# kvas7andy/unreal

Hardware: NVIDIA B200
Metric: maze env-steps/s incl. pixel-change+returns (higher is better)
Workload: dtype f32

## Files before the change

include/unreal_b200.h:

```cpp
#ifndef UNREAL_B200_H_
#define UNREAL_B200_H_

#include <stdint.h>

#ifdef __cplusplus
extern "C" {
#endif

#define UNREAL_OK 0
#define UNREAL_EINVAL (-1)
#define UNREAL_ECUDA (-2)
#define UNREAL_ESTATE (-3)
#define UNREAL_ENOMEM (-4)

#define UNREAL_F32 0
#define UNREAL_U8 1
#define UNREAL_BF16 2

#define UNREAL_MAZE_GRID 7
#define UNREAL_FRAME_HW 84
#define UNREAL_PC_CELLS 20
#define UNREAL_MT_WORDS 624

const char* unreal_last_error(void);
int unreal_abi_version(void);
int unreal_device_info(int* sm_count, int* cc_major, int* cc_minor);
int unreal_set_tunable(const char* name, int value);
int unreal_get_tunable(const char* name, int* value);

int unreal_maze_set_map(const char* map49_host);
int unreal_maze_get_layout(int* start_x, int* start_y, int* goal_x, int* goal_y, uint8_t* walls49_host);

int unreal_maze_reset(int32_t* pos , int32_t* last_action , float* last_reward ,
                      const uint8_t* mask , int n, void* stream);

int unreal_maze_step(int32_t* pos, const int32_t* action , const uint8_t* active,
                     float* reward , uint8_t* terminal , int32_t* last_action,
                     float* last_reward, void* obs, int obs_dtype, float* pc, uint64_t* frame_rec,
                     int n, int auto_reset, void* stream);

int unreal_maze_window(int32_t* pos, const int32_t* action, float* reward, uint8_t* terminal, int32_t* last_action,
                       float* last_reward, void* obs, int obs_dtype, float* pc, uint64_t* frame_rec, int n, int t,
                       int auto_reset, void* stream);

int unreal_maze_render(const int32_t* pos, void* obs, int obs_dtype, int m, void* stream);

int unreal_maze_pixel_change(const int32_t* pos0, const int32_t* pos1, float* pc, int m, void* stream);
int unreal_maze_pc_targets(const int32_t* pos0, const int32_t* pos1, const int32_t* len, const float* boot, float gamma_pc,
                           float* tgt, int t, int n, void* stream);

int unreal_pixel_change(const void* cur, const void* prev, int dtype, float* pc, int m, int h, int w,
                        int c, void* stream);
int unreal_selfcheck_arith(unsigned long long* mismatches, void* stream);
int unreal_subsample(const float* a, float* out, int m, int h, int w, int width, void* stream);
int unreal_pixel_change_stream(const void* frames, int dtype, float* pc, int s, int l, int h, int w,
                               int c, void* stream);

int unreal_nstep_returns(const float* r, const float* v, const uint8_t* term, const float* boot,
                         float gamma, float* out_R, float* out_adv, int t, int n, void* stream);
int unreal_sequence_returns(const float* r, const int32_t* len, const float* boot, float gamma,
                            float* out_R , int n, int l, void* stream);

int unreal_pc_targets(const float* pc, const uint8_t* term, const int32_t* len, const float* boot,
                      float gamma_pc, float* tgt, int t, int n, void* stream);

int unreal_mt_seed(uint32_t* mt, int32_t* mt_pos, const uint32_t* seeds , int n, void* stream);
int unreal_choose_action(uint32_t* mt, int32_t* mt_pos, const float* pi, const uint8_t* active,
                         int32_t* action, int n, int a, void* stream);
int unreal_mt_randint(uint32_t* mt, int32_t* mt_pos, uint32_t high, int32_t* out, int n, int k, void* stream);

typedef struct unreal_replay unreal_replay_t;
int unreal_replay_create(unreal_replay_t** out, int n_envs, int history_size);
int unreal_replay_destroy(unreal_replay_t* r);
int unreal_replay_reset(unreal_replay_t* r, void* stream);
int unreal_replay_add(unreal_replay_t* r, const uint64_t* frame_rec , void* stream);
int unreal_replay_state(unreal_replay_t* r, uint8_t* full, int32_t* count, int64_t* top,
                        int32_t* n_pos, int32_t* n_neg, void* stream);
int unreal_replay_copy(unreal_replay_t* r, int direction, uint64_t* rec, int64_t* top, int32_t* count,
                       int32_t* n_pos, int32_t* n_neg, void* stream);
int unreal_replay_sample_sequence(unreal_replay_t* r, uint32_t* mt, int32_t* mt_pos, int seq_len,
                                  int32_t* start, int32_t* len, uint64_t* rec, void* stream);
int unreal_replay_sample_rp(unreal_replay_t* r, uint32_t* mt, int32_t* mt_pos, int32_t* start,
                            uint64_t* rec, void* stream);
int unreal_frame_unpack(const uint64_t* rec, int m, int32_t* pos0, int32_t* pos1, int32_t* action,
                        float* reward, uint8_t* terminal, int32_t* last_action, float* last_reward,
                        uint8_t* valid, void* stream);

int unreal_frame_pack(const int32_t* action, const float* reward, const uint8_t* terminal,
                      const int32_t* last_action , const float* last_reward ,
                      const uint8_t* active , uint64_t* rec, int n, void* stream);
int unreal_replay_add_slots(unreal_replay_t* r, const uint64_t* frame_rec, int32_t* slot, void* stream);
int unreal_ring_store(void* payload, const void* src, const int32_t* slot, int n_envs, int history_size,
                      long long item_bytes, void* stream);
int unreal_rows_select(void* out, const void* src, const int64_t* idx, const uint8_t* mask, int n, long long item_bytes,
                       void* stream);
int unreal_replay_gather(unreal_replay_t* r, const void* payload, long long item_bytes, const int32_t* start,
                         const int32_t* len , int seq_len, int time_major, void* out, void* stream);

int unreal_rollout_lar(const int32_t* last_action, const float* last_reward, const float* objective, int n, int a, int g,
                       float* lar, void* stream);
int unreal_rollout_post(const float* reward, const uint8_t* terminal, const uint64_t* frame_rec, int n, uint8_t* active,
                        uint8_t* ended, uint64_t* last_rec, float* episode_reward, float* lstm_c, float* lstm_h,
// ... 124 lines not shown
```

unreal_b200/_lib.py:

```python
import ctypes
import os
from ctypes import POINTER, c_char_p, c_double, c_float, c_int, c_int32, c_int64, c_uint8, c_uint32, c_void_p

import torch

HERE = os.path.dirname(os.path.abspath(__file__))
LIB_PATH = os.path.join(HERE, "libunreal_b200.so")

OK = 0
F32 = 0
U8 = 1


class UnrealError(RuntimeError):
  pass


if not os.path.exists(LIB_PATH):
  raise ImportError(
      "%s is missing: build it with `python -m unreal_b200.build` (nvcc, sm_100a). "
      "unreal_b200 has no CPU fallback." % LIB_PATH)

lib = ctypes.CDLL(LIB_PATH)

P = c_void_p

SIGNATURES = {
    "unreal_last_error": (c_char_p, []),
    "unreal_abi_version": (c_int, []),
    "unreal_device_info": (c_int, [POINTER(c_int), POINTER(c_int), POINTER(c_int)]),
    "unreal_set_tunable": (c_int, [c_char_p, c_int]),
    "unreal_get_tunable": (c_int, [c_char_p, POINTER(c_int)]),
    "unreal_maze_set_map": (c_int, [c_char_p]),
    "unreal_maze_get_layout": (c_int, [POINTER(c_int)] * 4 + [POINTER(c_uint8)]),
    "unreal_maze_reset": (c_int, [P, P, P, P, c_int, P]),
    "unreal_maze_step": (c_int, [P, P, P, P, P, P, P, P, c_int, P, P, c_int, c_int, P]),
    "unreal_maze_window": (c_int, [P, P, P, P, P, P, P, c_int, P, P, c_int, c_int, c_int, P]),
    "unreal_maze_render": (c_int, [P, P, c_int, c_int, P]),
    "unreal_maze_pixel_change": (c_int, [P, P, P, c_int, P]),
    "unreal_maze_pc_targets": (c_int, [P, P, P, P, c_float, P, c_int, c_int, P]),
    "unreal_pixel_change": (c_int, [P, P, c_int, P, c_int, c_int, c_int, c_int, P]),
    "unreal_pixel_change_stream": (c_int, [P, c_int, P, c_int, c_int, c_int, c_int, c_int, P]),
    "unreal_selfcheck_arith": (c_int, [P, P]),
    "unreal_subsample": (c_int, [P, P, c_int, c_int, c_int, c_int, P]),
    "unreal_nstep_returns": (c_int, [P, P, P, P, c_float, P, P, c_int, c_int, P]),
    "unreal_sequence_returns": (c_int, [P, P, P, c_float, P, c_int, c_int, P]),
    "unreal_pc_targets": (c_int, [P, P, P, P, c_float, P, c_int, c_int, P]),
    "unreal_mt_seed": (c_int, [P, P, P, c_int, P]),
    "unreal_choose_action": (c_int, [P, P, P, P, P, c_int, c_int, P]),
    "unreal_mt_randint": (c_int, [P, P, c_uint32, P, c_int, c_int, P]),
    "unreal_replay_create": (c_int, [POINTER(c_void_p), c_int, c_int]),
    "unreal_replay_destroy": (c_int, [c_void_p]),
    "unreal_replay_reset": (c_int, [c_void_p, P]),
    "unreal_replay_add": (c_int, [c_void_p, P, P]),
    "unreal_replay_state": (c_int, [c_void_p, P, P, P, P, P, P]),
    "unreal_replay_copy": (c_int, [c_void_p, c_int, P, P, P, P, P, P]),
    "unreal_replay_sample_sequence": (c_int, [c_void_p, P, P, c_int, P, P, P, P]),
    "unreal_replay_sample_rp": (c_int, [c_void_p, P, P, P, P, P]),
    "unreal_frame_unpack": (c_int, [P, c_int, P, P, P, P, P, P, P, P, P]),
    "unreal_frame_pack": (c_int, [P, P, P, P, P, P, P, c_int, P]),
    "unreal_replay_add_slots": (c_int, [c_void_p, P, P, P]),
    "unreal_ring_store": (c_int, [P, P, P, c_int, c_int, c_int64, P]),
    "unreal_rows_select": (c_int, [P, P, P, P, c_int, c_int64, P]),
    "unreal_replay_gather": (c_int, [c_void_p, P, c_int64, P, P, c_int, c_int, P, P]),
    "unreal_rollout_lar": (c_int, [P, P, P, c_int, c_int, c_int, P, P]),
    "unreal_rollout_post": (c_int, [P, P, P, c_int, P, P, P, P, P, P, P, P]),
    "unreal_maze_eval_act": (c_int, [P, c_int, c_int, P, P, P, P, P, P, P, P, P, P, P, P, c_int, c_int, P, P, P, P, c_int64,
                                     c_int, c_int, P]),
    "unreal_grad_sumsq": (c_int, [P, c_int64, P, P]),
    "unreal_rmsprop_update": (c_int, [P, P, P, P, c_int64, P, c_float, c_float, c_float, c_float, c_float,
                                      c_float, P, P]),
    "unreal_rmsprop_update_dlr": (c_int, [P, P, P, P, c_int64, P, c_float, P, c_float, c_float, c_float,
                                          c_float, P, P]),
    "unreal_gemm_bf16": (c_int, [P, c_int64, c_int, P, c_int64, c_int, P, c_int64, c_int, P, P, c_int, c_int, c_int,
                                 c_int, c_int, c_int, P]),
    "unreal_im2col": (c_int, [P, c_int, P, c_int, c_int, c_int, c_int, c_int, c_int, c_int, P]),
    "unreal_col2im": (c_int, [P, c_int, P, c_int, P, c_int, c_int, c_int, c_int, c_int, c_int, c_int, c_int, P]),
    "unreal_lstm_cell_fwd": (c_int, [P, P, P, P, P, c_int, P]),
    "unreal_lstm_cell_fwd_ld": (c_int, [P, P, P, P, P, c_int, c_int, P]),
    "unreal_lstm_cell_act": (c_int, [P, P, P, P, P, c_int, P]),
    "unreal_lstm_cell_fwd_g16": (c_int, [P, P, P, P, P, c_int, c_int, P]),
    "unreal_lstm_cell_act_g16": (c_int, [P, P, P, P, P, c_int, P]),
    "unreal_lstm_cell_act_heads": (c_int, [P, P, P, P, c_int, P, P, P, P, c_int, P, P, P]),
    "unreal_lstm_cell_bwd_g16": (c_int, [P, P, P, P, P, P, P, c_int, P]),
    "unreal_lstm_step_fwd": (c_int, [P, c_int64, P, P, P, P, P, P, P, c_int, P, P, c_int, c_int, c_int, P]),
    "unreal_lstm_step_bwd": (c_int, [P, P, c_int64, P, P, P, P, P, P, P, c_int, c_int, P]),
    "unreal_lstm_cell_bwd": (c_int, [P, P, P, P, P, P, c_int, P]),
    "unreal_lstm_cell_bwd2": (c_int, [P, P, P, P, P, P, P, c_int, P]),
    "unreal_s2d_frames": (c_int, [P, c_int, P, c_int, P]),
    "unreal_conv_fwd": (c_int, [P, c_int, P, P, P, c_int, P]),
    "unreal_relu_grad": (c_int, [P, c_int, P, P, P, c_int64, c_int, c_int, P]),
    "unreal_conv1_wgrad": (c_int, [P, P, P, c_int, P]),
    "unreal_conv2_wgrad": (c_int, [P, P, P, c_int, P]),
# ... 118 lines not shown
```

unreal_b200/csrc/maze.cu:

```cuda
#include "common.cuh"
#include "maze_core.cuh"

namespace unreal {

__constant__ MazeLayout c_maze;
static MazeLayout h_maze;
static bool h_maze_ready = false;

static const char kReferenceMap[] =
    "--+---G"
    "--+-+++"
    "S-+---+"
    "--+++--"
    "--+-+--"
    "--+----"
    "-----++";

constexpr int kFrameElems = UNREAL_FRAME_HW * UNREAL_FRAME_HW * 3;
constexpr int kRowElems = UNREAL_FRAME_HW * 3;
constexpr int kPcElems = UNREAL_PC_CELLS * UNREAL_PC_CELLS;
constexpr int kThreads = 256;

struct StepArgs {
  int32_t* pos;
// ... 1 lines not shown
  const uint8_t* active;
  float* reward;
  uint8_t* terminal;
  int32_t* last_action;
  float* last_reward;
  void* obs;
  float* pc;
  uint64_t* rec;
  int n;
  int auto_reset;
};

struct EnvInfo {
  int rx, ry;
  int x0, y0, x1, y1;
  int live;
};

template <bool kStep>
__device__ __forceinline__ EnvInfo env_logic(const StepArgs& a, int e) {
  EnvInfo o;
  int x = a.pos[2 * e], y = a.pos[2 * e + 1];
  o.rx = x; o.ry = y; o.x0 = x; o.y0 = y; o.x1 = x; o.y1 = y; o.live = 1;
  if (!kStep) return o;
  if (a.active != nullptr && a.active[e] == 0) {
    o.live = 0;
    a.reward[e] = 0.f;
    a.terminal[e] = 0;
    if (a.rec) a.rec[e] = 0ull;
    return o;
  }
  int act = a.action[e];
  MazeStep s = maze_step_core(c_maze, x, y, act);
  int la = a.last_action[e];
  float lr = a.last_reward[e];
  if (a.rec) a.rec[e] = frame_pack(x, y, s.x1, s.y1, act, s.reward, s.terminal, la, (int)lr);
  a.reward[e] = (float)s.reward;
  a.terminal[e] = (uint8_t)s.terminal;
  o.x1 = s.x1; o.y1 = s.y1;
  if (s.terminal && a.auto_reset) {
    o.rx = c_maze.start_x; o.ry = c_maze.start_y;
    a.last_action[e] = 0;
    a.last_reward[e] = 0.f;
  } else {
    o.rx = s.x1; o.ry = s.y1;
    a.last_action[e] = act;
    a.last_reward[e] = (float)s.reward;
  }
  a.pos[2 * e] = o.rx;
  a.pos[2 * e + 1] = o.ry;
  return o;
}

__device__ __forceinline__ float4 pc_value4(int x0, int y0, int x1, int y1, int q) {
  int i = q / 5, j0 = (q - i * 5) * 4;
  bool moved = (x0 != x1) || (y0 != y1);
  int wy0 = pc_overlap(i, y0), wy1 = pc_overlap(i, y1);
  if (!moved || (wy0 | wy1) == 0) return make_float4(0.f, 0.f, 0.f, 0.f);
  float v[4];
#pragma unroll
  for (int u = 0; u < 4; ++u) {
    const float k = (float)(wy0 * pc_overlap(j0 + u, x0) + wy1 * pc_overlap(j0 + u, x1));
    const float q = k * 0x1.555556p-6f;
    v[u] = __fmaf_rn(__fmaf_rn(-q, 48.0f, k), 0x1.555556p-6f, q);
  }
  return make_float4(v[0], v[1], v[2], v[3]);
}
__device__ __forceinline__ void write_pc(float* pc, const EnvInfo& f, int q) {
  reinterpret_cast<float4*>(pc)[q] = pc_value4(f.x0, f.y0, f.x1, f.y1, q);
}

template <typename T> struct One;
template <> struct One<float> { static __device__ __forceinline__ float v() { return 1.0f; } };
template <> struct One<uint8_t> { static __device__ __forceinline__ uint8_t v() { return 255; } };

__device__ __forceinline__ void bulk_store(void* gdst, const void* ssrc, uint32_t bytes) {
  uint32_t s = (uint32_t)__cvta_generic_to_shared(ssrc);
  asm volatile("cp.async.bulk.global.shared::cta.bulk_group [%0], [%1], %2;" ::"l"(gdst), "r"(s), "r"(bytes)
               : "memory");
}
__device__ __forceinline__ void bulk_commit() { asm volatile("cp.async.bulk.commit_group;" ::: "memory"); }
template <int kPending>
__device__ __forceinline__ void bulk_wait_read() {
  asm volatile("cp.async.bulk.wait_group.read %0;" ::"n"(kPending) : "memory");
}
__device__ __forceinline__ void bulk_wait_all() { asm volatile("cp.async.bulk.wait_group 0;" ::: "memory"); }
__device__ __forceinline__ void fence_async_smem() { asm volatile("fence.proxy.async.shared::cta;" ::: "memory"); }

template <typename T>
__device__ __forceinline__ void set_agent(T* buf, int x, int y, int t, T val) {
  int j = t / 12, i = t - j * 12;
  buf[((12 * y + j) * UNREAL_FRAME_HW + 12 * x + i) * 3 + 1] = val;
}

template <typename T, int kBufs, bool kStep>
__global__ void __launch_bounds__(kThreads) maze_tma_kernel(StepArgs a) {
  extern __shared__ __align__(128) uint8_t smem_raw[];
  __shared__ EnvInfo s_info[2];
  T* bufs = reinterpret_cast<T*>(smem_raw);
  const int tid = threadIdx.x;
  constexpr uint32_t kFrameBytes = kFrameElems * sizeof(T);

  for (int i = tid; i < kFrameElems; i += kThreads) {
    int row = i / kRowElems;
    int f = i - row * kRowElems;
    int px = f / 3;
    int chn = f - px * 3;
    bool on = (chn == 0) && ((c_maze.wall_rows[row / 12] >> (px / 12)) & 1u);
    T v = on ? One<T>::v() : (T)0;
#pragma unroll
    for (int b = 0; b < kBufs; ++b) bufs[(size_t)b * kFrameElems + i] = v;
  }
  int drawn[kBufs];
#pragma unroll
  for (int b = 0; b < kBufs; ++b) drawn[b] = -1;
  fence_async_smem();
  __syncthreads();

  int it = 0;
  for (int e = blockIdx.x; e < a.n; e += gridDim.x, ++it) {
    const int b = it % kBufs;
    if (tid == 0) {
// ... 141 lines not shown
      __stcs(out + (size_t)g * kChunksPerGroup, band_value(m, c_maze.wall_rows[cy], cy == f.ry, f.rx));
    }
  }
}


struct WindowArgs {
  const int32_t* pos;
  const int32_t* last_action;
  const float* last_reward;
  const int32_t* action;
  float* reward;
  uint8_t* terminal;
  void* obs;
  float* pc;
  uint64_t* rec;
  int n, t, auto_reset;
};

struct MazeCursor { int x, y, la; float lr; };

__device__ __forceinline__ void cursor_advance(MazeCursor& c, const MazeStep& s, int act, int auto_reset) {
  if (s.terminal && auto_reset) { c.x = c_maze.start_x; c.y = c_maze.start_y; c.la = 0; c.lr = 0.f; }
  else { c.x = s.x1; c.y = s.y1; c.la = act; c.lr = (float)s.reward; }
}

__device__ __forceinline__ EnvInfo window_logic(const WindowArgs& a, int e, int t, int lane) {
  const int mine = (lane <= t) ? a.action[(size_t)lane * a.n + e] : 0;
  MazeCursor c{a.pos[2 * e], a.pos[2 * e + 1], a.last_action[e], a.last_reward[e]};
  for (int s = 0; s < t; ++s) {
    const int act = __shfl_sync(0xffffffffu, mine, s);
    cursor_advance(c, maze_step_core(c_maze, c.x, c.y, act), act, a.auto_reset);
  }
  const int act = __shfl_sync(0xffffffffu, mine, t);
  const MazeStep st = maze_step_core(c_maze, c.x, c.y, act);
  const size_t b = (size_t)t * a.n + e;
  if (lane == 0) {
    if (a.rec) a.rec[b] = frame_pack(c.x, c.y, st.x1, st.y1, act, st.reward, st.terminal, c.la, (int)c.lr);
    a.reward[b] = (float)st.reward;
    a.terminal[b] = (uint8_t)st.terminal;
  }
  EnvInfo o;
  o.x0 = c.x; o.y0 = c.y; o.x1 = st.x1; o.y1 = st.y1; o.live = 1;
  const bool reset = st.terminal && a.auto_reset;
  o.rx = reset ? c_maze.start_x : st.x1;
  o.ry = reset ? c_maze.start_y : st.y1;
  return o;
}

__global__ void maze_window_state_kernel(int32_t* pos, int32_t* last_action, float* last_reward,
                                         const int32_t* __restrict__ action, int n, int t, int auto_reset) {
  const int e = blockIdx.x * blockDim.x + threadIdx.x;
  if (e >= n) return;
  MazeCursor c{pos[2 * e], pos[2 * e + 1], last_action[e], last_reward[e]};
  for (int s = 0; s < t; ++s) {
    const int act = action[(size_t)s * n + e];
    cursor_advance(c, maze_step_core(c_maze, c.x, c.y, act), act, auto_reset);
  }
  pos[2 * e] = c.x; pos[2 * e + 1] = c.y; last_action[e] = c.la; last_reward[e] = c.lr;
}

template <typename T, int kThreads>
__global__ void __launch_bounds__(kThreads) maze_window_cta_kernel(WindowArgs a) {
  __shared__ EnvInfo s_info;
  constexpr int kChunksPerGroup = 63;
  constexpr int R = kThreads / kChunksPerGroup;
  constexpr int G = Chunk<T>::kGroupsPerBand;
  constexpr int kGroups = G * UNREAL_MAZE_GRID;
  const int tid = threadIdx.x;
  const size_t b = blockIdx.x;
  const int t = (int)(b / a.n), e = (int)(b - (size_t)t * a.n);
  if (tid < 32) {
    const EnvInfo f = window_logic(a, e, t, tid);
    if (tid == 0) s_info = f;
  }
  const int gsub = tid / kChunksPerGroup;
  const int c = tid - gsub * kChunksPerGroup;
  const ChunkMasks m = make_masks<T>(c);
  __syncthreads();
  const EnvInfo f = s_info;
  if (a.pc != nullptr && tid >= kThreads - kPcElems / 4) write_pc(a.pc + b * kPcElems, f, tid - (kThreads - kPcElems / 4));
  if (a.obs == nullptr || gsub >= R) return;
  uint4* out = reinterpret_cast<uint4*>(reinterpret_cast<T*>(a.obs) + b * kFrameElems) + c;
#pragma unroll
  for (int j = 0; j < (kGroups + R - 1) / R; ++j) {
    const int g = gsub + R * j;
    if (g < kGroups) {
      const int cy = g / G;
      __stcs(out + (size_t)g * kChunksPerGroup, band_value(m, c_maze.wall_rows[cy], cy == f.ry, f.rx));
    }
  }
}

template <typename T, int kWarps>
__global__ void __launch_bounds__(kWarps * 32) maze_window_warp_kernel(WindowArgs a) {
  const int lane = threadIdx.x & 31;
  const size_t b = (size_t)blockIdx.x * kWarps + (threadIdx.x >> 5);
  if (b >= (size_t)a.n * a.t) return;
  const int t = (int)(b / a.n), e = (int)(b - (size_t)t * a.n);
  const EnvInfo f = window_logic(a, e, t, lane);
  if (a.pc != nullptr) {
    float* pc = a.pc + b * kPcElems;
#pragma unroll
    for (int q = lane; q < kPcElems / 4; q += 32) write_pc(pc, f, q);
  }
  if (a.obs == nullptr) return;
  constexpr int G = Chunk<T>::kGroupsPerBand;
  constexpr int kChunksPerGroup = 63;
  const ChunkMasks m0 = make_masks<T>(lane);
  const ChunkMasks m1 = make_masks<T>(lane + 32);
  const bool has1 = lane + 32 < kChunksPerGroup;
// ... 94 lines not shown
  for (int q = 0; q < 6; ++q) {
    const int base = (2 * q) % 3;
    uint32_t wl[4], ag[4];
#pragma unroll
    for (int k = 0; k < 4; ++k) {
      const int c0 = (base + 2 * k) % 3, c1 = (base + 2 * k + 1) % 3;
      wl[k] = (c0 == 0 ? 0x3f80u : 0u) | (c1 == 0 ? 0x3f800000u : 0u);
      ag[k] = (c0 == 1 ? 0x3f80u : 0u) | (c1 == 1 ? 0x3f800000u : 0u);
    }
#pragma unroll
    for (int h = 0; h < 2; ++h) {
      if (kind[h] < 0) continue;
      const uint32_t mw = (kind[h] & 1) ? 0xffffffffu : 0u, ma = (kind[h] & 2) ? 0xffffffffu : 0u;
      __stcs(out + q * 441 + tid + h * 256, make_uint4((wl[0] & mw) | (ag[0] & ma), (wl[1] & mw) | (ag[1] & ma),
                                                       (wl[2] & mw) | (ag[2] & ma), (wl[3] & mw) | (ag[3] & ma)));
    }
  }
}

__global__ void __launch_bounds__(128) maze_pc_pairs_kernel(const int32_t* __restrict__ p0,
                                                            const int32_t* __restrict__ p1, float* pc, int m) {
  int idx = blockIdx.x * blockDim.x + threadIdx.x;
  int e = idx / (kPcElems / 4), q = idx - e * (kPcElems / 4);
  if (e >= m) return;
  EnvInfo f;
  f.x0 = p0[2 * e]; f.y0 = p0[2 * e + 1]; f.x1 = p1[2 * e]; f.y1 = p1[2 * e + 1];
  f.rx = f.ry = 0; f.live = 1;
  write_pc(pc + (size_t)e * kPcElems, f, q);
}

__global__ void __launch_bounds__(128) maze_pc_targets_kernel(const int2* __restrict__ p0, const int2* __restrict__ p1,
                                                              const int32_t* __restrict__ len, const float4* __restrict__ boot,
                                                              float g, float4* __restrict__ tgt, int T, int N) {
  const size_t per_t = (size_t)N * (kPcElems / 4);
  const size_t idx = (size_t)blockIdx.x * 128 + threadIdx.x;
  if (idx >= per_t) return;
  const int n = (int)(idx / (kPcElems / 4)), q = (int)(idx - (size_t)n * (kPcElems / 4));
  const int n_t = len ? max(0, min(len[n], T)) : T;
  const float4 zero = make_float4(0.f, 0.f, 0.f, 0.f);
  float4 R = boot[idx];
  for (int t = T - 1; t >= n_t; --t) __stcs(tgt + (size_t)t * per_t + idx, zero);
#pragma unroll 4
  for (int t = n_t - 1; t >= 0; --t) {
    const int2 a = __ldg(p0 + (size_t)t * N + n), b = __ldg(p1 + (size_t)t * N + n);
    const float4 pc = pc_value4(a.x, a.y, b.x, b.y, q);
    R.x = __fadd_rn(pc.x, __fmul_rn(g, R.x));
    R.y = __fadd_rn(pc.y, __fmul_rn(g, R.y));
    R.z = __fadd_rn(pc.z, __fmul_rn(g, R.z));
    R.w = __fadd_rn(pc.w, __fmul_rn(g, R.w));
    __stcs(tgt + (size_t)t * per_t + idx, R);
  }
}

__global__ void maze_reset_kernel(int32_t* pos, int32_t* last_action, float* last_reward, const uint8_t* mask,
                                  int n) {
  int e = blockIdx.x * blockDim.x + threadIdx.x;
  if (e >= n || (mask != nullptr && mask[e] == 0)) return;
  pos[2 * e] = c_maze.start_x;
  pos[2 * e + 1] = c_maze.start_y;
  if (last_action) last_action[e] = 0;
  if (last_reward) last_reward[e] = 0.f;
}

static int ensure_map() {
  if (h_maze_ready) return UNREAL_OK;
  return unreal_maze_set_map(nullptr);
}

template <bool kStep>
static int launch_render(const StepArgs& a, int obs_dtype, cudaStream_t st) {
  if (a.n == 0) return UNREAL_OK;
  const int sms = sm_count();
  if (sms <= 0) return UNREAL_ECUDA;
  if (obs_dtype == UNREAL_BF16) {
    maze_s2d_kernel<kStep><<<a.n, 256, 0, st>>>(a);
    UNREAL_LAUNCH_CHECK("maze_s2d_kernel");
    return UNREAL_OK;
  }
  int variant = get_tunable("maze_render_variant", -1);
  if (variant < 0) variant = (a.obs == nullptr || obs_dtype == UNREAL_U8) ? 2 : 0;
  if (a.obs == nullptr && variant == 1) variant = 0;
  if (variant == 2) {
    const int warps = get_tunable("maze_warps_per_cta", 4);
    if (obs_dtype == UNREAL_F32) {
      maze_warp_kernel<float, kStep, 4><<<(a.n + 3) / 4, 128, 0, st>>>(a);
    } else if (warps == 16) {
      maze_warp_kernel<uint8_t, kStep, 16><<<(a.n + 15) / 16, 512, 0, st>>>(a);
    } else if (warps == 8) {
      maze_warp_kernel<uint8_t, kStep, 8><<<(a.n + 7) / 8, 256, 0, st>>>(a);
    } else if (warps == 2) {
      maze_warp_kernel<uint8_t, kStep, 2><<<(a.n + 1) / 2, 64, 0, st>>>(a);
    } else {
      maze_warp_kernel<uint8_t, kStep, 4><<<(a.n + 3) / 4, 128, 0, st>>>(a);
    }
    UNREAL_LAUNCH_CHECK("maze_warp_kernel");
    return UNREAL_OK;
  }
  if (variant == 0) {
    if (obs_dtype == UNREAL_F32) {
      if (get_tunable("maze_cta_threads", 256) == 512) maze_cta_kernel<float, kStep, 512><<<a.n, 512, 0, st>>>(a);
      else maze_cta_kernel<float, kStep, 256><<<a.n, 256, 0, st>>>(a);
    } else {
      if (get_tunable("maze_cta_threads", 256) == 512) maze_cta_kernel<uint8_t, kStep, 512><<<a.n, 512, 0, st>>>(a);
      else maze_cta_kernel<uint8_t, kStep, 256><<<a.n, 256, 0, st>>>(a);
    }
    UNREAL_LAUNCH_CHECK("maze_cta_kernel");
// ... 86 lines not shown
  UNREAL_LAUNCH_CHECK("maze_reset_kernel");
  return UNREAL_OK;
}

extern "C" int unreal_maze_step(int32_t* pos, const int32_t* action, const uint8_t* active, float* reward,
                                uint8_t* terminal, int32_t* last_action, float* last_reward, void* obs,
                                int obs_dtype, float* pc, uint64_t* frame_rec, int n, int auto_reset,
                                void* stream) {
  UNREAL_REQUIRE(n >= 0, "unreal_maze_step: n < 0");
  UNREAL_REQUIRE(pos && action && reward && terminal && last_action && last_reward,
                 "unreal_maze_step: pos/action/reward/terminal/last_action/last_reward must be non-null");
  UNREAL_REQUIRE(obs_dtype == UNREAL_F32 || obs_dtype == UNREAL_U8 || obs_dtype == UNREAL_BF16,
                 "unreal_maze_step: bad obs_dtype %d", obs_dtype);
  UNREAL_REQUIRE(aligned16(obs) && aligned16(pc), "unreal_maze_step: obs and pc must be 16-byte aligned");
  int rc = ensure_map();
  if (rc) return rc;
  StepArgs a{pos, action, active, reward, terminal, last_action, last_reward, obs, pc, frame_rec, n, auto_reset};
  return launch_render<true>(a, obs_dtype, as_stream(stream));
}

extern "C" int unreal_maze_render(const int32_t* pos, void* obs, int obs_dtype, int m, void* stream) {
  UNREAL_REQUIRE(pos && obs && m >= 0, "unreal_maze_render: null argument or m < 0");
  UNREAL_REQUIRE(obs_dtype == UNREAL_F32 || obs_dtype == UNREAL_U8 || obs_dtype == UNREAL_BF16,
                 "unreal_maze_render: bad obs_dtype %d", obs_dtype);
  UNREAL_REQUIRE(aligned16(obs), "unreal_maze_render: obs must be 16-byte aligned");
  int rc = ensure_map();
  if (rc) return rc;
  StepArgs a{const_cast<int32_t*>(pos), nullptr, nullptr, nullptr, nullptr, nullptr, nullptr, obs, nullptr, nullptr, m, 0};
  return launch_render<false>(a, obs_dtype, as_stream(stream));
}

extern "C" int unreal_maze_pixel_change(const int32_t* pos0, const int32_t* pos1, float* pc, int m, void* stream) {
  UNREAL_REQUIRE(pos0 && pos1 && pc && m >= 0, "unreal_maze_pixel_change: null argument or m < 0");
  UNREAL_REQUIRE(aligned16(pc), "unreal_maze_pixel_change: pc must be 16-byte aligned");
  if (m == 0) return UNREAL_OK;
  long long threads = (long long)m * (kPcElems / 4);
  maze_pc_pairs_kernel<<<(unsigned)((threads + 127) / 128), 128, 0, as_stream(stream)>>>(pos0, pos1, pc, m);
  UNREAL_LAUNCH_CHECK("maze_pc_pairs_kernel");
  return UNREAL_OK;
}

extern "C" int unreal_maze_pc_targets(const int32_t* pos0, const int32_t* pos1, const int32_t* len, const float* boot,
                                      float gamma_pc, float* tgt, int t, int n, void* stream) {
  UNREAL_REQUIRE(t >= 0 && n >= 0, "unreal_maze_pc_targets: negative size");
  if (t == 0 || n == 0) return UNREAL_OK;
  UNREAL_REQUIRE(pos0 && pos1 && boot && tgt, "unreal_maze_pc_targets: pos0, pos1, boot and tgt must be non-null");
  UNREAL_REQUIRE(aligned16(boot) && aligned16(tgt) && (reinterpret_cast<uintptr_t>(pos0) & 7u) == 0 &&
                 (reinterpret_cast<uintptr_t>(pos1) & 7u) == 0, "unreal_maze_pc_targets: alignment (16 bytes; cells 8)");
  const long long cols = (long long)n * (kPcElems / 4);
  maze_pc_targets_kernel<<<(unsigned)((cols + 127) / 128), 128, 0, as_stream(stream)>>>(
      reinterpret_cast<const int2*>(pos0), reinterpret_cast<const int2*>(pos1), len, reinterpret_cast<const float4*>(boot),
      gamma_pc, reinterpret_cast<float4*>(tgt), t, n);
  UNREAL_LAUNCH_CHECK("maze_pc_targets_kernel");
  return UNREAL_OK;
}

extern "C" int unreal_maze_window(int32_t* pos, const int32_t* action, float* reward, uint8_t* terminal, int32_t* last_action,
                                  float* last_reward, void* obs, int obs_dtype, float* pc, uint64_t* frame_rec, int n, int t,
                                  int auto_reset, void* stream) {
  UNREAL_REQUIRE(n >= 0 && t >= 0, "unreal_maze_window: negative size");
  UNREAL_REQUIRE(t <= 32, "unreal_maze_window: at most 32 steps per window (got %d)", t);
  UNREAL_REQUIRE(pos && action && reward && terminal && last_action && last_reward,
                 "unreal_maze_window: pos/action/reward/terminal/last_action/last_reward must be non-null");
  UNREAL_REQUIRE(obs_dtype == UNREAL_F32 || obs_dtype == UNREAL_U8, "unreal_maze_window: obs_dtype must be f32 or u8");
  UNREAL_REQUIRE(aligned16(obs) && aligned16(pc), "unreal_maze_window: obs and pc must be 16-byte aligned");
  UNREAL_REQUIRE((long long)n * t < 2147483647LL / 4, "unreal_maze_window: window too large for one launch");
  int rc = ensure_map();
  if (rc) return rc;
  if (n == 0 || t == 0) return UNREAL_OK;
  cudaStream_t st = as_stream(stream);
  WindowArgs a{pos, last_action, last_reward, action, reward, terminal, obs, pc, frame_rec, n, t, auto_reset};
  const long long items = (long long)n * t;
  int variant = get_tunable("maze_render_variant", -1);
  if (variant < 0 || variant == 1) variant = (obs == nullptr || obs_dtype == UNREAL_U8) ? 3 : 0;
  if (variant == 3) {
    const int warps = get_tunable("maze_warps_per_cta", 8);
    if (obs_dtype == UNREAL_F32) maze_window_env_kernel<float, 4><<<(n + 3) / 4, 128, 0, st>>>(a, pos, last_action, last_reward);
    else if (warps == 4) maze_window_env_kernel<uint8_t, 4><<<(n + 3) / 4, 128, 0, st>>>(a, pos, last_action, last_reward);
    else if (warps == 2) maze_window_env_kernel<uint8_t, 2><<<(n + 1) / 2, 64, 0, st>>>(a, pos, last_action, last_reward);
    else if (warps == 1) maze_window_env_kernel<uint8_t, 1><<<n, 32, 0, st>>>(a, pos, last_action, last_reward);
    else maze_window_env_kernel<uint8_t, 8><<<(n + 7) / 8, 256, 0, st>>>(a, pos, last_action, last_reward);
    UNREAL_LAUNCH_CHECK("maze_window_env_kernel");
    return UNREAL_OK;
  }
  if (variant == 2) {
    if (obs_dtype == UNREAL_F32) maze_window_warp_kernel<float, 4><<<(unsigned)((items + 3) / 4), 128, 0, st>>>(a);
    else if (get_tunable("maze_warps_per_cta", 4) == 8) maze_window_warp_kernel<uint8_t, 8><<<(unsigned)((items + 7) / 8), 256, 0, st>>>(a);
    else maze_window_warp_kernel<uint8_t, 4><<<(unsigned)((items + 3) / 4), 128, 0, st>>>(a);
    UNREAL_LAUNCH_CHECK("maze_window_warp_kernel");
  } else {
    if (obs_dtype == UNREAL_F32) maze_window_cta_kernel<float, 256><<<(unsigned)items, 256, 0, st>>>(a);
    else maze_window_cta_kernel<uint8_t, 256><<<(unsigned)items, 256, 0, st>>>(a);
    UNREAL_LAUNCH_CHECK("maze_window_cta_kernel");
  }
  maze_window_state_kernel<<<(n + 127) / 128, 128, 0, st>>>(pos, last_action, last_reward, action, n, t, auto_reset);
  UNREAL_LAUNCH_CHECK("maze_window_state_kernel");
  return UNREAL_OK;
}
```

unreal_b200/kernels.py:

```python
import ctypes

import torch

from . import _lib
from ._lib import call, ptr, stream_ptr

FRAME = 84
PC = 20
MT_WORDS = 624


def maze_set_map(map49=None):
  call("unreal_maze_set_map", None if map49 is None else map49.encode())


def maze_layout():
  v = [ctypes.c_int() for _ in range(4)]
  walls = (ctypes.c_uint8 * 49)()
  call("unreal_maze_get_layout", *[ctypes.byref(x) for x in v], walls)
  return (v[0].value, v[1].value), (v[2].value, v[3].value), bytes(walls)


class MazeState(object):

# ... 49 lines not shown
    raise _lib.UnrealError("actions must be [T, %d]" % state.n)
  if reward is None:
    reward = torch.empty(t, n, dtype=torch.float32, device=dev)
  if terminal is None:
    terminal = torch.empty(t, n, dtype=torch.uint8, device=dev)
  if obs is not None and (obs.numel() != t * n * FRAME * FRAME * 3 or obs.dtype not in (torch.float32, torch.uint8)):
    raise _lib.UnrealError("obs must hold [T,N,84,84,3] float32 or uint8")
  if pc is not None and (pc.numel() != t * n * PC * PC or pc.dtype != torch.float32):
    raise _lib.UnrealError("pc must be float32 [T,N,20,20]")
  call("unreal_maze_window", ptr(state.pos, torch.int32), ptr(actions, torch.int32, "actions"), ptr(reward, torch.float32),
       ptr(terminal, torch.uint8), ptr(state.last_action, torch.int32), ptr(state.last_reward, torch.float32), ptr(obs),
       _lib.dtype_tag(obs) if obs is not None else _lib.F32, ptr(pc), ptr(frame_rec, torch.int64, "frame_rec"), n, t,
       1 if auto_reset else 0, stream_ptr())
  return reward, terminal


def obs_shape(dtype):
  if dtype == torch.int32:
    return (2,)
  return (6, 441, 8) if dtype == torch.bfloat16 else (FRAME, FRAME, 3)


def maze_render(pos, out=None, dtype=torch.float32):
  m = pos.shape[0]
  if (out is not None and out.dtype == torch.int32) or (out is None and dtype == torch.int32):
    if out is None:
      return pos.reshape(m, 2).clone()
    out.copy_(pos.view_as(out))
    return out
  if out is None:
    out = torch.empty(m, *obs_shape(dtype), dtype=dtype, device=pos.device)
  call("unreal_maze_render", ptr(pos, torch.int32, "pos"), ptr(out), _lib.dtype_tag(out), m, stream_ptr())
  return out


def maze_pixel_change(pos0, pos1, out=None):
  m = pos0.shape[0]
  if out is None:
    out = torch.empty(m, PC, PC, dtype=torch.float32, device=pos0.device)
  call("unreal_maze_pixel_change", ptr(pos0, torch.int32), ptr(pos1, torch.int32), ptr(out, torch.float32), m,
       stream_ptr())
  return out


def maze_pc_targets(pos0, pos1, length, boot, gamma_pc, out=None):
  t, n = pos0.shape[0], pos0.shape[1]
  if out is None:
    out = torch.empty(t, n, PC, PC, dtype=torch.float32, device=pos0.device)
  call("unreal_maze_pc_targets", ptr(pos0, torch.int32), ptr(pos1, torch.int32), ptr(length, torch.int32),
       ptr(boot, torch.float32), float(gamma_pc), ptr(out, torch.float32), t, n, stream_ptr())
  return out


def pixel_change(cur, prev, out=None):
  m, h, w, c = cur.shape
  if out is None:
    out = torch.empty(m, (h - 4) // 4, (w - 4) // 4, dtype=torch.float32, device=cur.device)
  if prev.shape != cur.shape or prev.dtype != cur.dtype:
    raise _lib.UnrealError("cur and prev must have the same shape and dtype")
  call("unreal_pixel_change", ptr(cur), ptr(prev), _lib.dtype_tag(cur), ptr(out, torch.float32), m, h, w, c,
       stream_ptr())
  return out


def pixel_change_stream(frames, out=None):
  s, l1, h, w, c = frames.shape
  if out is None:
    out = torch.empty(s, l1 - 1, (h - 4) // 4, (w - 4) // 4, dtype=torch.float32, device=frames.device)
  call("unreal_pixel_change_stream", ptr(frames), _lib.dtype_tag(frames), ptr(out, torch.float32), s, l1 - 1, h, w,
       c, stream_ptr())
  return out


def selfcheck_arith():
  out = torch.zeros(2, dtype=torch.int64, device="cuda")
  call("unreal_selfcheck_arith", ptr(out), stream_ptr())
  return tuple(int(x) for x in out.tolist())


def subsample(a, width, out=None):
  m, h, w = a.shape
  if out is None:
    out = torch.empty(m, h // width, w // width, dtype=torch.float32, device=a.device)
  call("unreal_subsample", ptr(a, torch.float32, "a"), ptr(out, torch.float32, "out"), m, h, w, int(width), stream_ptr())
  return out


def nstep_returns(r, v, term, boot, gamma, out_R=None, out_adv=None):
  t, n = r.shape
  if out_R is None:
    out_R = torch.empty_like(r)
  if v is not None and out_adv is None:
    out_adv = torch.empty_like(r)
  call("unreal_nstep_returns", ptr(r, torch.float32), ptr(v, torch.float32), ptr(term, torch.uint8),
       ptr(boot, torch.float32), float(gamma), ptr(out_R, torch.float32), ptr(out_adv, torch.float32), t, n,
       stream_ptr())
  return out_R, out_adv


def sequence_returns(r, length, boot, gamma, out=None):
  n, l = r.shape
  if out is None:
    out = torch.empty_like(r)
  call("unreal_sequence_returns", ptr(r, torch.float32), ptr(length, torch.int32), ptr(boot, torch.float32),
       float(gamma), ptr(out, torch.float32), n, l, stream_ptr())
  return out
# ... 795 lines not shown
```

unreal_b200/train/rollout.py:

```python
import torch

from .. import _lib
from .. import kernels as K


class RolloutTargets(object):
  def __init__(self, num_envs, rollout_len=20, gamma=0.99, gamma_pc=0.9, obs_dtype=torch.float32,
               device="cuda:0", auto_reset=True, use_graphs=True, window_kernel=None):
    self.n = int(num_envs)
    self.t = int(rollout_len)
    self.gamma = float(gamma)
    self.gamma_pc = float(gamma_pc)
    self.device = torch.device(device)
    self.auto_reset = auto_reset
    self.use_graphs = use_graphs
    self.window_kernel = (self.t <= 32) if window_kernel is None else bool(window_kernel)
    if self.window_kernel and self.t > 32:
      raise _lib.UnrealError("the window kernel covers at most 32 rollout steps")
    d, n, t = self.device, self.n, self.t
    with torch.cuda.device(d):
      self.state = K.MazeState(n, d)
    self.actions = torch.zeros(t, n, dtype=torch.int32, device=d)
    self.values = torch.zeros(t, n, dtype=torch.float32, device=d)
    self.boot_value = torch.zeros(n, dtype=torch.float32, device=d)
    self.boot_q = torch.zeros(n, 20, 20, dtype=torch.float32, device=d)
    self.obs = torch.empty(t, n, 84, 84, 3, dtype=obs_dtype, device=d)
    self.pc = torch.empty(t, n, 20, 20, dtype=torch.float32, device=d)
    self.reward = torch.empty(t, n, dtype=torch.float32, device=d)
    self.terminal = torch.empty(t, n, dtype=torch.uint8, device=d)
    self.frame_rec = torch.empty(t, n, dtype=torch.int64, device=d)
    self.R = torch.empty(t, n, dtype=torch.float32, device=d)
    self.adv = torch.empty(t, n, dtype=torch.float32, device=d)
    self.pc_tgt = torch.empty(t, n, 20, 20, dtype=torch.float32, device=d)
    self._graphs = None
    self._h_in = None
    self._h_out = None
    self._copy_stream = None
    self.host_graph = True
    self._host_graph = None

  @property
  def launches_per_pass(self):
    return ((1 if self.obs.dtype == torch.uint8 else 2) if self.window_kernel else self.t) + 2

  def _steps(self):
    if self.window_kernel:
      K.maze_window(self.state, self.actions, obs=self.obs, pc=self.pc, reward=self.reward, terminal=self.terminal,
                    frame_rec=self.frame_rec, auto_reset=self.auto_reset)
      return
    for t in range(self.t):
      K.maze_step(self.state, self.actions[t], obs=self.obs[t], pc=self.pc[t], reward=self.reward[t],
                  terminal=self.terminal[t], frame_rec=self.frame_rec[t], auto_reset=self.auto_reset)

  def _returns(self):
    K.nstep_returns(self.reward, self.values, self.terminal, self.boot_value, self.gamma, self.R, self.adv)

  def _pc_targets(self):
    K.pc_targets(self.pc, self.terminal, None, self.boot_q, self.gamma_pc, self.pc_tgt)

  def _capture(self):
    torch.cuda.synchronize(self.device)
    self._steps(); self._returns(); self._pc_targets()
    K.maze_reset(self.state)
    torch.cuda.synchronize(self.device)
    graphs = []
    for fn in (self._steps, self._returns, self._pc_targets):
      g = torch.cuda.CUDAGraph()
      with _lib.graph_capture(g):
        fn()
      graphs.append(g)
    self._graphs = graphs

  def run_device(self, events=None):
    with torch.cuda.device(self.device):
      if self.use_graphs and self._graphs is None:
        self._capture()
      phases = ([g.replay for g in self._graphs] if self.use_graphs
                else [self._steps, self._returns, self._pc_targets])
      if events is not None:
        events[0].record()
      for i, ph in enumerate(phases):
        ph()
        if events is not None:
          events[i + 1].record()

  def _ensure_host(self):
    if self._h_in is None:
      t, n = self.t, self.n
      pin = dict(pin_memory=True)
      self._h_in = dict(actions=torch.zeros(t, n, dtype=torch.int32, **pin),
                        values=torch.zeros(t, n, dtype=torch.float32, **pin),
                        boot_value=torch.zeros(n, dtype=torch.float32, **pin),
                        boot_q=torch.zeros(n, 20, 20, dtype=torch.float32, **pin))
      self._h_out = dict(reward=torch.zeros(t, n, dtype=torch.float32, **pin),
                         terminal=torch.zeros(t, n, dtype=torch.uint8, **pin),
                         R=torch.zeros(t, n, dtype=torch.float32, **pin),
                         adv=torch.zeros(t, n, dtype=torch.float32, **pin))

  @property
  def h2d_bytes_per_pass(self):
    self._ensure_host()
    return sum(v.numel() * v.element_size() for v in self._h_in.values())

  @property
  def d2h_bytes_per_pass(self):
    self._ensure_host()
    return sum(v.numel() * v.element_size() for v in self._h_out.values())

  def host_inputs(self):
    self._ensure_host()
    return {k: v.numpy() for k, v in self._h_in.items()}

  def run_host(self, actions=None, values=None, boot_value=None, boot_q=None):
    self._ensure_host()
    hi, ho = self._h_in, self._h_out
    for name, arr in (("actions", actions), ("values", values), ("boot_value", boot_value), ("boot_q", boot_q)):
      if arr is None:
        continue
      t = torch.as_tensor(arr)
      if t.data_ptr() != hi[name].data_ptr():
        hi[name].copy_(t)
    with torch.cuda.device(self.device):
      if self.use_graphs and self._graphs is None:
        self._capture()
      if self._copy_stream is None:
        self._copy_stream = torch.cuda.Stream(self.device)
        self._ev = [torch.cuda.Event() for _ in range(5)]
      main = torch.cuda.current_stream()
      if self.use_graphs and self.host_graph:
        if self._host_graph is None:
          self._pipeline(main)
          main.synchronize()
          g = torch.cuda.CUDAGraph()
          with _lib.graph_capture(g):
            self._pipeline(torch.cuda.current_stream(), replay_graphs=False)
          self._host_graph = g
        else:
          self._host_graph.replay()
      else:
        self._pipeline(main)
      main.synchronize()
    return {k: v.numpy() for k, v in self._h_out.items()}

  def _pipeline(self, main, replay_graphs=True):
    hi, ho = self._h_in, self._h_out
    side = self._copy_stream
    ev_start, ev_in, ev_k1, ev_k3, ev_out = self._ev
    phases = ([g.replay for g in self._graphs] if (self.use_graphs and replay_graphs)
              else [self._steps, self._returns, self._pc_targets])
    ev_start.record(main)
    self.actions.copy_(hi["actions"], non_blocking=True)
    side.wait_event(ev_start)
    with torch.cuda.stream(side):
      self.values.copy_(hi["values"], non_blocking=True)
      self.boot_value.copy_(hi["boot_value"], non_blocking=True)
      self.boot_q.copy_(hi["boot_q"], non_blocking=True)
      ev_in.record(side)
    phases[0]()
    ev_k1.record(main)
    with torch.cuda.stream(side):
      side.wait_event(ev_k1)
      ho["reward"].copy_(self.reward, non_blocking=True)
      ho["terminal"].copy_(self.terminal, non_blocking=True)
    main.wait_event(ev_in)
    phases[1]()
    ev_k3.record(main)
    with torch.cuda.stream(side):
      side.wait_event(ev_k3)
      ho["R"].copy_(self.R, non_blocking=True)
      ho["adv"].copy_(self.adv, non_blocking=True)
      ev_out.record(side)
    phases[2]()
    main.wait_event(ev_out)
```

Before: 78.52 million.

## Fuse n-step returns and pixel-change targets into one rollout-targets kernel

Replaces the separate n-step returns and pc-targets launches with one kernel. Its first blocks compute returns and advantages, and the remaining blocks rebuild pixel-change targets from the packed frame records instead of reading the stored per-step pc tensor. It also computes pixel-change overlap for four columns at once with packed byte arithmetic, switches pc writes to streaming stores, and preloads up to 32 actions in the window kernel. This removes one launch and a large pc read, in exchange for recomputing pc values and a hard 32-step limit in the unrolled window loop.

```diff
diff --git a/include/unreal_b200.h b/include/unreal_b200.h
--- a/include/unreal_b200.h
+++ b/include/unreal_b200.h
@@ -48,6 +48,9 @@
 int unreal_maze_pixel_change(const int32_t* pos0, const int32_t* pos1, float* pc, int m, void* stream);
 int unreal_maze_pc_targets(const int32_t* pos0, const int32_t* pos1, const int32_t* len, const float* boot, float gamma_pc,
                            float* tgt, int t, int n, void* stream);
+int unreal_maze_rollout_targets(const uint64_t* rec, const float* values, const float* boot_value, const float* boot_q,
+                                float gamma, float gamma_pc, float* out_R, float* out_adv, float* pc_tgt, int t, int n,
+                                void* stream);
 
 int unreal_pixel_change(const void* cur, const void* prev, int dtype, float* pc, int m, int h, int w,
                         int c, void* stream);
diff --git a/unreal_b200/_lib.py b/unreal_b200/_lib.py
--- a/unreal_b200/_lib.py
+++ b/unreal_b200/_lib.py
@@ -39,6 +39,7 @@
     "unreal_maze_render": (c_int, [P, P, c_int, c_int, P]),
     "unreal_maze_pixel_change": (c_int, [P, P, P, c_int, P]),
     "unreal_maze_pc_targets": (c_int, [P, P, P, P, c_float, P, c_int, c_int, P]),
+    "unreal_maze_rollout_targets": (c_int, [P, P, P, P, c_float, c_float, P, P, P, c_int, c_int, P]),
     "unreal_pixel_change": (c_int, [P, P, c_int, P, c_int, c_int, c_int, c_int, P]),
     "unreal_pixel_change_stream": (c_int, [P, c_int, P, c_int, c_int, c_int, c_int, c_int, P]),
     "unreal_selfcheck_arith": (c_int, [P, P]),
diff --git a/unreal_b200/csrc/maze.cu b/unreal_b200/csrc/maze.cu
--- a/unreal_b200/csrc/maze.cu
+++ b/unreal_b200/csrc/maze.cu
@@ -77,22 +77,28 @@
   return o;
 }
 
+__device__ __forceinline__ uint32_t pc_overlap4(int j0, int c) {
+  const int s = 8 * (3 * c - 1 - j0);
+  const uint32_t run = 0x02040402u;
+  return s >= 0 ? (s < 32 ? run << s : 0u) : (s > -32 ? run >> -s : 0u);
+}
+
 __device__ __forceinline__ float4 pc_value4(int x0, int y0, int x1, int y1, int q) {
-  int i = q / 5, j0 = (q - i * 5) * 4;
-  bool moved = (x0 != x1) || (y0 != y1);
-  int wy0 = pc_overlap(i, y0), wy1 = pc_overlap(i, y1);
-  if (!moved || (wy0 | wy1) == 0) return make_float4(0.f, 0.f, 0.f, 0.f);
+  const int i = q / 5, j0 = (q - i * 5) * 4;
+  const bool moved = (x0 != x1) || (y0 != y1);
+  const uint32_t k4 = moved ? (uint32_t)pc_overlap(i, y0) * pc_overlap4(j0, x0) + (uint32_t)pc_overlap(i, y1) * pc_overlap4(j0, x1)
+                            : 0u;
   float v[4];
 #pragma unroll
   for (int u = 0; u < 4; ++u) {
-    const float k = (float)(wy0 * pc_overlap(j0 + u, x0) + wy1 * pc_overlap(j0 + u, x1));
+    const float k = (float)((k4 >> (8 * u)) & 0xffu);
     const float q = k * 0x1.555556p-6f;
     v[u] = __fmaf_rn(__fmaf_rn(-q, 48.0f, k), 0x1.555556p-6f, q);
   }
   return make_float4(v[0], v[1], v[2], v[3]);
 }
 __device__ __forceinline__ void write_pc(float* pc, const EnvInfo& f, int q) {
-  reinterpret_cast<float4*>(pc)[q] = pc_value4(f.x0, f.y0, f.x1, f.y1, q);
+  __stcs(reinterpret_cast<float4*>(pc) + q, pc_value4(f.x0, f.y0, f.x1, f.y1, q));
 }
 
 template <typename T> struct One;
@@ -340,11 +346,13 @@
                                          const int32_t* __restrict__ action, int n, int t, int auto_reset) {
   const int e = blockIdx.x * blockDim.x + threadIdx.x;
   if (e >= n) return;
+  int acts[32];
+#pragma unroll
+  for (int s = 0; s < 32; ++s) acts[s] = (s < t) ? __ldg(action + (size_t)s * n + e) : 0;
   MazeCursor c{pos[2 * e], pos[2 * e + 1], last_action[e], last_reward[e]};
-  for (int s = 0; s < t; ++s) {
-    const int act = action[(size_t)s * n + e];
-    cursor_advance(c, maze_step_core(c_maze, c.x, c.y, act), act, auto_reset);
-  }
+#pragma unroll
+  for (int s = 0; s < 32; ++s)
+    if (s < t) cursor_advance(c, maze_step_core(c_maze, c.x, c.y, acts[s]), acts[s], auto_reset);
   pos[2 * e] = c.x; pos[2 * e + 1] = c.y; last_action[e] = c.la; last_reward[e] = c.lr;
 }
 
@@ -545,6 +553,86 @@
   }
 }
 
+constexpr int kTgtThreads = 128;
+constexpr int kTgtChunk = 10;
+constexpr int kTgtPcChunk = 5;
+constexpr int kTgtPcPer = 2;
+constexpr int kTgtPcCols = kPcElems / 4 / kTgtPcPer;
+
+__device__ __forceinline__ uint64_t valid_record(uint64_t r) { return frame_valid(r) ? r : 0ull; }
+
+__global__ void __launch_bounds__(kTgtThreads, 8) maze_rollout_targets_kernel(
+    const uint64_t* __restrict__ rec, const float* __restrict__ values, const float* __restrict__ boot_value,
+    const float4* __restrict__ boot_q, float gamma, float gamma_pc, float* __restrict__ out_R,
+    float* __restrict__ out_adv, float4* __restrict__ tgt, int T, int N, int ret_blocks) {
+  if ((int)blockIdx.x < ret_blocks) {
+    const int n = blockIdx.x * kTgtThreads + threadIdx.x;
+    if (n >= N) return;
+    float R = boot_value[n];
+    for (int hi = T; hi > 0; hi -= kTgtChunk) {
+      const int lo = hi - kTgtChunk;
+      int rr[kTgtChunk];
+      float vv[kTgtChunk];
+#pragma unroll
+      for (int k = 0; k < kTgtChunk; ++k) {
+        if (lo + k >= 0) {
+          const size_t o = (size_t)(lo + k) * N + n;
+          const uint64_t r = valid_record(__ldg(rec + o));
+          rr[k] = (frame_reward(r) & 0xff) | (frame_terminal(r) << 8);
+          vv[k] = __ldcs(values + o);
+        }
+      }
+#pragma unroll
+      for (int k = kTgtChunk - 1; k >= 0; --k) {
+        if (lo + k >= 0) {
+          const size_t o = (size_t)(lo + k) * N + n;
+          R = (rr[k] & 0x100) ? 0.f : R;
+          R = __fadd_rn((float)(int8_t)rr[k], __fmul_rn(gamma, R));
+          __stcs(out_R + o, R);
+          __stcs(out_adv + o, __fsub_rn(R, vv[k]));
+        }
+      }
+    }
+    return;
+  }
+  const size_t per_t = (size_t)N * (kPcElems / 4);
+  const size_t col = (size_t)(blockIdx.x - ret_blocks) * kTgtThreads + threadIdx.x;
+  if (col >= (size_t)N * kTgtPcCols) return;
+  const int n = (int)(col / kTgtPcCols), q0 = (int)(col - (size_t)n * kTgtPcCols);
+  const float4 zero = make_float4(0.f, 0.f, 0.f, 0.f);
+  float4 R[kTgtPcPer];
+#pragma unroll
+  for (int p = 0; p < kTgtPcPer; ++p) R[p] = boot_q[(size_t)n * (kPcElems / 4) + q0 + p * kTgtPcCols];
+  for (int hi = T; hi > 0; hi -= kTgtPcChunk) {
+    const int lo = hi - kTgtPcChunk;
+    uint32_t cc[kTgtPcChunk];
+#pragma unroll
+    for (int k = 0; k < kTgtPcChunk; ++k) {
+      if (lo + k >= 0) {
+        const uint64_t r = valid_record(__ldg(rec + (size_t)(lo + k) * N + n));
+        cc[k] = (uint32_t)(r & 0xffffu) | ((uint32_t)frame_terminal(r) << 16);
+      }
+    }
+#pragma unroll
+    for (int k = kTgtPcChunk - 1; k >= 0; --k) {
+      if (lo + k >= 0) {
+        const uint64_t r = cc[k];
+#pragma unroll
+        for (int p = 0; p < kTgtPcPer; ++p) {
+          const int q = q0 + p * kTgtPcCols;
+          const float4 pc = pc_value4(frame_x0(r), frame_y0(r), frame_x1(r), frame_y1(r), q);
+          if (r >> 16) R[p] = zero;
+          R[p].x = __fadd_rn(pc.x, __fmul_rn(gamma_pc, R[p].x));
+          R[p].y = __fadd_rn(pc.y, __fmul_rn(gamma_pc, R[p].y));
+          R[p].z = __fadd_rn(pc.z, __fmul_rn(gamma_pc, R[p].z));
+          R[p].w = __fadd_rn(pc.w, __fmul_rn(gamma_pc, R[p].w));
+          __stcs(tgt + (size_t)(lo + k) * per_t + (size_t)n * (kPcElems / 4) + q, R[p]);
+        }
+      }
+    }
+  }
+}
+
 __global__ void maze_reset_kernel(int32_t* pos, int32_t* last_action, float* last_reward, const uint8_t* mask,
                                   int n) {
   int e = blockIdx.x * blockDim.x + threadIdx.x;
@@ -737,6 +825,25 @@
       reinterpret_cast<const int2*>(pos0), reinterpret_cast<const int2*>(pos1), len, reinterpret_cast<const float4*>(boot),
       gamma_pc, reinterpret_cast<float4*>(tgt), t, n);
   UNREAL_LAUNCH_CHECK("maze_pc_targets_kernel");
+  return UNREAL_OK;
+}
+
+extern "C" int unreal_maze_rollout_targets(const uint64_t* rec, const float* values, const float* boot_value,
+                                           const float* boot_q, float gamma, float gamma_pc, float* out_R, float* out_adv,
+                                           float* pc_tgt, int t, int n, void* stream) {
+  UNREAL_REQUIRE(t >= 0 && n >= 0, "unreal_maze_rollout_targets: negative size");
+  if (t == 0 || n == 0) return UNREAL_OK;
+  UNREAL_REQUIRE(rec && values && boot_value && boot_q && out_R && out_adv && pc_tgt,
+                 "unreal_maze_rollout_targets: null argument");
+  UNREAL_REQUIRE(aligned16(boot_q) && aligned16(pc_tgt) && (reinterpret_cast<uintptr_t>(rec) & 7u) == 0,
+                 "unreal_maze_rollout_targets: alignment (boot_q / pc_tgt 16 bytes; rec 8)");
+  const long long cols = (long long)n * kTgtPcCols;
+  const int ret_blocks = (n + kTgtThreads - 1) / kTgtThreads;
+  const long long blocks = ret_blocks + (cols + kTgtThreads - 1) / kTgtThreads;
+  maze_rollout_targets_kernel<<<(unsigned)blocks, kTgtThreads, 0, as_stream(stream)>>>(
+      rec, values, boot_value, reinterpret_cast<const float4*>(boot_q), gamma, gamma_pc, out_R, out_adv,
+      reinterpret_cast<float4*>(pc_tgt), t, n, ret_blocks);
+  UNREAL_LAUNCH_CHECK("maze_rollout_targets_kernel");
   return UNREAL_OK;
 }
 
diff --git a/unreal_b200/kernels.py b/unreal_b200/kernels.py
--- a/unreal_b200/kernels.py
+++ b/unreal_b200/kernels.py
@@ -125,6 +125,21 @@
   return out
 
 
+def maze_rollout_targets(rec, values, boot_value, boot_q, gamma, gamma_pc, R=None, adv=None, pc_tgt=None):
+  t, n = rec.shape
+  if R is None:
+    R = torch.empty(t, n, dtype=torch.float32, device=rec.device)
+  if adv is None:
+    adv = torch.empty(t, n, dtype=torch.float32, device=rec.device)
+  if pc_tgt is None:
+    pc_tgt = torch.empty(t, n, PC, PC, dtype=torch.float32, device=rec.device)
+  call("unreal_maze_rollout_targets", ptr(rec, torch.int64, "rec"), ptr(values, torch.float32, "values"),
+       ptr(boot_value, torch.float32, "boot_value"), ptr(boot_q, torch.float32, "boot_q"), float(gamma), float(gamma_pc),
+       ptr(R, torch.float32, "R"), ptr(adv, torch.float32, "adv"), ptr(pc_tgt, torch.float32, "pc_tgt"), t, n,
+       stream_ptr())
+  return R, adv, pc_tgt
+
+
 def pixel_change(cur, prev, out=None):
   m, h, w, c = cur.shape
   if out is None:
diff --git a/unreal_b200/train/rollout.py b/unreal_b200/train/rollout.py
--- a/unreal_b200/train/rollout.py
+++ b/unreal_b200/train/rollout.py
@@ -41,7 +41,7 @@
 
   @property
   def launches_per_pass(self):
-    return ((1 if self.obs.dtype == torch.uint8 else 2) if self.window_kernel else self.t) + 2
+    return ((1 if self.obs.dtype == torch.uint8 else 2) if self.window_kernel else self.t) + 1
 
   def _steps(self):
     if self.window_kernel:
@@ -52,19 +52,17 @@
       K.maze_step(self.state, self.actions[t], obs=self.obs[t], pc=self.pc[t], reward=self.reward[t],
                   terminal=self.terminal[t], frame_rec=self.frame_rec[t], auto_reset=self.auto_reset)
 
-  def _returns(self):
-    K.nstep_returns(self.reward, self.values, self.terminal, self.boot_value, self.gamma, self.R, self.adv)
-
-  def _pc_targets(self):
-    K.pc_targets(self.pc, self.terminal, None, self.boot_q, self.gamma_pc, self.pc_tgt)
+  def _targets(self):
+    K.maze_rollout_targets(self.frame_rec, self.values, self.boot_value, self.boot_q, self.gamma, self.gamma_pc,
+                           self.R, self.adv, self.pc_tgt)
 
   def _capture(self):
     torch.cuda.synchronize(self.device)
-    self._steps(); self._returns(); self._pc_targets()
+    self._steps(); self._targets()
     K.maze_reset(self.state)
     torch.cuda.synchronize(self.device)
     graphs = []
-    for fn in (self._steps, self._returns, self._pc_targets):
+    for fn in (self._steps, self._targets):
       g = torch.cuda.CUDAGraph()
       with _lib.graph_capture(g):
         fn()
@@ -75,14 +73,15 @@
     with torch.cuda.device(self.device):
       if self.use_graphs and self._graphs is None:
         self._capture()
-      phases = ([g.replay for g in self._graphs] if self.use_graphs
-                else [self._steps, self._returns, self._pc_targets])
+      phases = [g.replay for g in self._graphs] if self.use_graphs else [self._steps, self._targets]
       if events is not None:
         events[0].record()
       for i, ph in enumerate(phases):
         ph()
         if events is not None:
           events[i + 1].record()
+      if events is not None:
+        events[3].record()
 
   def _ensure_host(self):
     if self._h_in is None:
@@ -145,9 +144,9 @@
   def _pipeline(self, main, replay_graphs=True):
     hi, ho = self._h_in, self._h_out
     side = self._copy_stream
-    ev_start, ev_in, ev_k1, ev_k3, ev_out = self._ev
+    ev_start, ev_in, ev_k1, ev_tg, ev_out = self._ev
     phases = ([g.replay for g in self._graphs] if (self.use_graphs and replay_graphs)
-              else [self._steps, self._returns, self._pc_targets])
+              else [self._steps, self._targets])
     ev_start.record(main)
     self.actions.copy_(hi["actions"], non_blocking=True)
     side.wait_event(ev_start)
@@ -164,11 +163,10 @@
       ho["terminal"].copy_(self.terminal, non_blocking=True)
     main.wait_event(ev_in)
     phases[1]()
-    ev_k3.record(main)
+    ev_tg.record(main)
     with torch.cuda.stream(side):
-      side.wait_event(ev_k3)
+      side.wait_event(ev_tg)
       ho["R"].copy_(self.R, non_blocking=True)
       ho["adv"].copy_(self.adv, non_blocking=True)
       ev_out.record(side)
-    phases[2]()
     main.wait_event(ev_out)
```

After: 81.73 million (median of 6 runs). 4.1% higher.
